# DefTruth/CUDA-Learn-Notes

Measured on NVIDIA H100. Metric: hgemm_tflops, higher is better.
Workload: dtype f16 (fp32 accumulate)

## Files before the change

### cuda-learn-notes_b200/csrc/hgemm_wgmma.cu

```cuda
#include "abi_common.cuh"
#include "ptx.cuh"

namespace b200k {

namespace gemm {
constexpr int BM = 128, BN = 256, STAGES = 4, THREADS = 384, GROUP_M = 16;
constexpr int STG_BYTES = 16384;
}

template <int DT_, bool A_MN_, bool B_MN_>
struct GemmCfg {
  static constexpr int DT = DT_;
  static constexpr bool A_MN = A_MN_, B_MN = B_MN_;
  static constexpr int ES = DT == 2 ? 4 : 2;
  static constexpr int BK = 128 / ES;
  static constexpr int KSTEP = DT == 2 ? 8 : 16;
  static constexpr int A_BYTES = gemm::BM * BK * ES;
  static constexpr int B_BYTES = gemm::BN * BK * ES;
  static constexpr int STAGE_BYTES = A_BYTES + B_BYTES;
  static constexpr int SMEM_BYTES = gemm::STAGES * STAGE_BYTES + 2 * gemm::STG_BYTES + 1024 + 2 * gemm::STAGES * 8;
  static_assert(!(DT == 2 && (A_MN || B_MN)), "tf32 wgmma reads K-major operands only");
  static_assert(SMEM_BYTES <= 232448, "more shared memory than an H100 block may use");
};

template <class Cfg>
__device__ __forceinline__ void gemm_mma_kblock(float* d, uint32_t sA, uint32_t sB, int cw) {
  constexpr int STEPS = Cfg::BK / Cfg::KSTEP;
#pragma unroll
  for (int k = 0; k < STEPS; ++k) {
    const uint64_t da = Cfg::A_MN ? wgmma_desc(sA + cw * 64 * Cfg::BK * Cfg::ES + k * 2048, 64 * Cfg::BK * Cfg::ES, 1024)
                                  : wgmma_desc(sA + cw * 64 * 128 + k * 32, 16, 1024);
    const uint64_t db = Cfg::B_MN ? wgmma_desc(sB + k * 2048, 64 * Cfg::BK * Cfg::ES, 1024) : wgmma_desc(sB + k * 32, 16, 1024);
    wgmma_ss<Cfg::DT, 256, Cfg::A_MN, Cfg::B_MN>(d, da, db, 1);
  }
}

template <class Cfg>
__device__ __forceinline__ void gemm_store_tile(const float* d, const CUtensorMap* tmC, uint32_t stg, int cw, int row0,
                                                int col0) {
  constexpr int SLICES = Cfg::DT == 2 ? 4 : 2, JS = 32 / SLICES, JB = JS / 2;
  const int t = threadIdx.x & 127, lane = t & 31, warp = t / 32;
  const bool leader = t == 0;
#pragma unroll
  for (int sl = 0; sl < SLICES; ++sl) {
    if (leader) tma_store_wait_read<0>();
    named_bar_sync(1 + cw, 128);
    if constexpr (Cfg::DT == 2) {
      const int q = lane & 3;
#pragma unroll
      for (int jj = 0; jj < JS; ++jj) {
        const int j = sl * JS + jj;
#pragma unroll
        for (int h = 0; h < 2; ++h) {
          const int r = warp * 16 + 8 * h + lane / 4;
          const int chunk = 2 * (jj % JB) + q / 2;
          const uint32_t a = stg + (jj / JB) * 8192 + r * 128 + ((chunk ^ (r & 7)) << 4) + (q & 1) * 8;
          asm volatile("st.shared.v2.f32 [%0], {%1, %2};" ::"r"(a), "f"(d[4 * j + 2 * h]), "f"(d[4 * j + 2 * h + 1])
                       : "memory");
        }
      }
    } else {
      const int m = lane / 8, r = warp * 16 + 8 * (m & 1) + (lane & 7);
#pragma unroll
      for (int jj = 0; jj < JS; jj += 2) {
        const int j = sl * JS + jj, chunk = jj % JB + (m >> 1);
        const uint32_t a = stg + (jj / JB) * 8192 + r * 128 + ((chunk ^ (r & 7)) << 4);
        uint32_t p[4];
#pragma unroll
        for (int i = 0; i < 4; ++i)
          p[i] = Cfg::DT == 1 ? pack_bf162(d[4 * j + 2 * i], d[4 * j + 2 * i + 1])
                              : pack_half2(d[4 * j + 2 * i], d[4 * j + 2 * i + 1]);
        stmatrix_x4(a, p[0], p[1], p[2], p[3]);
      }
    }
    fence_proxy_async_smem();
    named_bar_sync(1 + cw, 128);
    if (leader) {
      const int c = col0 + sl * (gemm::BN / SLICES);
      tma_store_2d(tmC, stg, c, row0);
      tma_store_2d(tmC, stg + 8192, c + 128 / Cfg::ES, row0);
      tma_store_commit();
    }
  }
}

template <class Cfg>
__global__ void __launch_bounds__(gemm::THREADS, 1)
    hgemm_wgmma_kernel(const __grid_constant__ CUtensorMap tmA, const __grid_constant__ CUtensorMap tmB,
                       const __grid_constant__ CUtensorMap tmC, int K, int tiles_m, int tiles_n) {
  using namespace gemm;
  extern __shared__ uint8_t smem_raw[];
  const uint32_t base = (smem_u32(smem_raw) + 1023) & ~1023u;
  const uint32_t stg0 = base + STAGES * Cfg::STAGE_BYTES;
  const uint32_t full0 = stg0 + 2 * STG_BYTES, empty0 = full0 + STAGES * 8;
  const int wg = threadIdx.x / 128;

  const int tile = blockIdx.x, width = GROUP_M * tiles_n, g = tile / width, first_m = g * GROUP_M;
  const int gsz = min(tiles_m - first_m, GROUP_M);
  const int tm = first_m + (tile % width) % gsz, tn = (tile % width) / gsz;
  const int nkb = (K + Cfg::BK - 1) / Cfg::BK;

  if (threadIdx.x == 0) {
    for (int s = 0; s < STAGES; ++s) {
      mbar_init(full0 + 8 * s, 1);
      mbar_init(empty0 + 8 * s, 2);
    }
    fence_mbar_init();
  }
  __syncthreads();

  if (wg == 0) {
    if (threadIdx.x == 0) {
      tma_prefetch_desc(&tmA);
      tma_prefetch_desc(&tmB);
      for (int kb = 0; kb < nkb; ++kb) {
        const int s = kb % STAGES;
        if (kb >= STAGES) mbar_wait_nocall(empty0 + 8 * s, ((kb / STAGES) - 1) & 1);
        const uint32_t bar = full0 + 8 * s, sA = base + s * Cfg::STAGE_BYTES, sB = sA + Cfg::A_BYTES;
        mbar_arrive_expect_tx(bar, Cfg::STAGE_BYTES);
        if constexpr (Cfg::A_MN) {
#pragma unroll
          for (int c = 0; c < BM / 64; ++c)
            tma_load_2d(sA + c * 64 * Cfg::BK * Cfg::ES, &tmA, bar, tm * BM + c * 64, kb * Cfg::BK, kPolicyEvictNormal);
        } else {
          tma_load_2d(sA, &tmA, bar, kb * Cfg::BK, tm * BM, kPolicyEvictNormal);
        }
        if constexpr (Cfg::B_MN) {
#pragma unroll
          for (int c = 0; c < BN / 64; ++c)
            tma_load_2d(sB + c * 64 * Cfg::BK * Cfg::ES, &tmB, bar, tn * BN + c * 64, kb * Cfg::BK, kPolicyEvictNormal);
        } else {
          tma_load_2d(sB, &tmB, bar, kb * Cfg::BK, tn * BN, kPolicyEvictNormal);
        }
      }
    }
    return;
  }

  const int cw = wg - 1, t = threadIdx.x & 127;
  const bool leader = t == 0;
  if (leader) tma_prefetch_desc(&tmC);
  float d[128];
#pragma unroll
  for (int i = 0; i < 128; ++i) d[i] = 0.f;
  for (int kb = 0; kb < nkb; ++kb) {
    const int s = kb % STAGES;
    mbar_wait_nocall(full0 + 8 * s, (kb / STAGES) & 1);
    const uint32_t sA = base + s * Cfg::STAGE_BYTES, sB = sA + Cfg::A_BYTES;
    fence_regs<128>(d);
    wgmma_fence();
    gemm_mma_kblock<Cfg>(d, sA, sB, cw);
    wgmma_commit();
    wgmma_wait<1>();
    fence_regs<128>(d);
    if (kb > 0 && leader) mbar_arrive(empty0 + 8 * ((kb - 1) % STAGES));
  }
  wgmma_wait<0>();
  fence_regs<128>(d);
  gemm_store_tile<Cfg>(d, &tmC, stg0 + cw * STG_BYTES, cw, tm * BM + cw * 64, tn * BN);
  if (leader) tma_store_wait_all<0>();
}

template <class Cfg>
static int launch_gemm(const void* A, const void* B, void* C, int64_t M, int64_t N, int64_t K, cudaStream_t s,
                       const DeviceInfo& di) {
  using namespace gemm;
  auto tmap = [](CUtensorMap* m, const void* p, int64_t rows, int64_t cols, uint32_t box_rows, uint32_t box_cols) {
    const uint64_t dims[2] = {uint64_t(cols), uint64_t(rows)}, strides[1] = {uint64_t(cols) * Cfg::ES};
    const uint32_t box[2] = {box_cols, box_rows};
    return make_tmap(m, p, Cfg::ES, 2, dims, strides, box);
  };
  CUtensorMap tmA, tmB, tmC;
  int rc = Cfg::A_MN ? tmap(&tmA, A, K, M, Cfg::BK, 64) : tmap(&tmA, A, M, K, BM, Cfg::BK);
  if (rc) return rc;
  rc = Cfg::B_MN ? tmap(&tmB, B, K, N, Cfg::BK, 64) : tmap(&tmB, B, N, K, BN, Cfg::BK);
  if (rc) return rc;
  if ((rc = tmap(&tmC, C, M, N, 64, 128 / Cfg::ES))) return rc;
  const int64_t tiles_m = (M + BM - 1) / BM, tiles_n = (N + BN - 1) / BN, tiles = tiles_m * tiles_n;
  if (tiles > INT32_MAX) return set_error(B200K_ESHAPE, "GEMM too large: %lld tiles", (long long)tiles);
  auto kern = hgemm_wgmma_kernel<Cfg>;
  if ((rc = ensure_dynamic_smem(reinterpret_cast<const void*>(kern), di.device, Cfg::SMEM_BYTES))) return rc;
  kern<<<unsigned(tiles), THREADS, Cfg::SMEM_BYTES, s>>>(tmA, tmB, tmC, int(K), int(tiles_m), int(tiles_n));
  B200K_CHECK_CUDA(cudaGetLastError());
  return B200K_OK;
}

template <int DT>
static int gemm_dispatch(const char* who, const void* A, const void* B, void* C, int64_t M, int64_t N, int64_t K,
                         int b_is_nk, int variant, void* stream, int a_is_km = 0) {
  constexpr int PACK = (DT == 2) ? 4 : 8;
  if (!A || !B || !C) return set_error(B200K_EARG, "%s: null pointer", who);
  if (reinterpret_cast<uintptr_t>(C) & 15) return set_error(B200K_EALIGN, "%s: C (%p) must be 16-byte aligned", who, C);
  if (M < 1 || N < 1 || K < 1 || M > INT32_MAX || N > INT32_MAX || K > INT32_MAX)
    return set_error(B200K_ESHAPE, "%s: M,N,K must be in [1, 2^31) (got %lld,%lld,%lld)", who, (long long)M, (long long)N,
                     (long long)K);
  if ((K % PACK) || (N % PACK))
    return set_error(B200K_ESHAPE, "%s: K and N must be multiples of %d (16-byte rows), got K=%lld N=%lld", who, PACK,
                     (long long)K, (long long)N);
  if (a_is_km && DT == 2) return set_error(B200K_EDTYPE, "%s: A stored as [K,M] is built for f16 / bf16 only", who);
  if (a_is_km && (M % PACK))
    return set_error(B200K_ESHAPE, "%s: M must be a multiple of %d when A is stored as [K,M]", who, PACK);
  const int v = variant & 0xff;
  if (v < B200K_HGEMM_AUTO || v > B200K_HGEMM_2CTA_512x256)
    return set_error(B200K_EARG, "%s: variant %d unknown", who, v);
  DeviceInfo di;
  int rc = get_device_info(&di);
  if (rc) return rc;
  cudaStream_t s = static_cast<cudaStream_t>(stream);
  const bool nn = (b_is_nk == 0);
  if constexpr (DT == 2) {
    if (!nn) return launch_gemm<GemmCfg<2, false, false>>(A, B, C, M, N, K, s, di);
    void* bt = nullptr;
    B200K_CHECK_CUDA(cudaMallocAsync(&bt, size_t(K) * size_t(N) * 4, s));
    rc = b200k_mat_transpose_f32(B, bt, K, N, stream);
    if (!rc) rc = launch_gemm<GemmCfg<2, false, false>>(A, bt, C, M, N, K, s, di);
    cudaError_t e = cudaFreeAsync(bt, s);
    if (!rc && e != cudaSuccess) rc = set_error(B200K_ECUDA, "cudaFreeAsync failed: %s", cudaGetErrorString(e));
    return rc;
  } else {
    if (a_is_km)
      return nn ? launch_gemm<GemmCfg<DT, true, true>>(A, B, C, M, N, K, s, di)
                : launch_gemm<GemmCfg<DT, true, false>>(A, B, C, M, N, K, s, di);
    return nn ? launch_gemm<GemmCfg<DT, false, true>>(A, B, C, M, N, K, s, di)
              : launch_gemm<GemmCfg<DT, false, false>>(A, B, C, M, N, K, s, di);
  }
}

}

extern "C" int b200k_hgemm_f16(const void* A, const void* B, void* C, int64_t M, int64_t N, int64_t K, int b_is_nk,
                               int variant, void* stream) {
  return b200k::gemm_dispatch<0>("b200k_hgemm_f16", A, B, C, M, N, K, b_is_nk, variant, stream);
}

extern "C" int b200k_gemm_ex(const void* A, const void* B, void* C, int64_t M, int64_t N, int64_t K, int a_is_km, int b_is_nk,
                             int dtype, int variant, void* stream) {
  switch (dtype) {
    case B200K_F16: return b200k::gemm_dispatch<0>("b200k_gemm_ex(f16)", A, B, C, M, N, K, b_is_nk, variant, stream, a_is_km);
    case B200K_BF16: return b200k::gemm_dispatch<1>("b200k_gemm_ex(bf16)", A, B, C, M, N, K, b_is_nk, variant, stream, a_is_km);
    case B200K_F32: return b200k::gemm_dispatch<2>("b200k_gemm_ex(tf32)", A, B, C, M, N, K, b_is_nk, variant, stream, a_is_km);
    default: return b200k::set_error(B200K_EDTYPE, "b200k_gemm_ex: dtype %d not supported (f16, bf16, f32-as-tf32)", dtype);
  }
}

extern "C" int b200k_gemm(const void* A, const void* B, void* C, int64_t M, int64_t N, int64_t K, int b_is_nk, int dtype,
                          int variant, void* stream) {
  switch (dtype) {
    case B200K_F16: return b200k::gemm_dispatch<0>("b200k_gemm(f16)", A, B, C, M, N, K, b_is_nk, variant, stream);
    case B200K_BF16: return b200k::gemm_dispatch<1>("b200k_gemm(bf16)", A, B, C, M, N, K, b_is_nk, variant, stream);
    case B200K_F32: return b200k::gemm_dispatch<2>("b200k_gemm(tf32)", A, B, C, M, N, K, b_is_nk, variant, stream);
    default: return b200k::set_error(B200K_EDTYPE, "b200k_gemm: dtype %d not supported (f16, bf16, f32-as-tf32)", dtype);
  }
}
```

### cuda-learn-notes_b200/csrc/ptx.cuh

```cuda
#pragma once
#include <cstdint>
#include <cuda.h>
#include <cuda_bf16.h>
#include <cuda_fp16.h>
#include <cuda_runtime.h>

namespace b200k {

#ifndef B200K_SPIN_LIMIT_CYCLES
#define B200K_SPIN_LIMIT_CYCLES (10LL * 1000 * 1000 * 1000)
#endif

__device__ __forceinline__ uint32_t smem_u32(const void* p) {
  return static_cast<uint32_t>(__cvta_generic_to_shared(p));
}
__device__ __forceinline__ void named_bar_sync(uint32_t id, uint32_t nthreads) {
  asm volatile("bar.sync %0, %1;" ::"r"(id), "r"(nthreads) : "memory");
}

__device__ __forceinline__ void mbar_init(uint32_t bar, uint32_t count) {
  asm volatile("mbarrier.init.shared::cta.b64 [%0], %1;" ::"r"(bar), "r"(count) : "memory");
}
__device__ __forceinline__ void fence_mbar_init() {
  asm volatile("fence.mbarrier_init.release.cluster;" ::: "memory");
}
__device__ __forceinline__ void fence_proxy_async_smem() {
  asm volatile("fence.proxy.async.shared::cta;" ::: "memory");
}
__device__ __forceinline__ void mbar_arrive(uint32_t bar) {
  asm volatile("mbarrier.arrive.shared::cta.b64 _, [%0];" ::"r"(bar) : "memory");
}
__device__ __forceinline__ void mbar_arrive_expect_tx(uint32_t bar, uint32_t bytes) {
  asm volatile("mbarrier.arrive.expect_tx.shared::cta.b64 _, [%0], %1;" ::"r"(bar), "r"(bytes) : "memory");
}
__device__ __forceinline__ uint32_t mbar_try_wait(uint32_t bar, uint32_t parity) {
  uint32_t ok;
  asm volatile(
      "{\n\t"
      ".reg .pred P1;\n\t"
      "mbarrier.try_wait.parity.shared::cta.b64 P1, [%1], %2;\n\t"
      "selp.u32 %0, 1, 0, P1;\n\t"
      "}"
      : "=r"(ok)
      : "r"(bar), "r"(parity)
      : "memory");
  return ok;
}
static __device__ __noinline__ void mbar_timeout_trap(uint32_t bar, uint32_t parity) {
  printf("[b200k] mbarrier wait timed out: block (%d,%d) thread %d bar 0x%x parity %u\n", blockIdx.x, blockIdx.y,
         threadIdx.x, bar, parity);
  __trap();
}
__device__ __forceinline__ void mbar_wait(uint32_t bar, uint32_t parity) {
  if (mbar_try_wait(bar, parity)) return;
  long long t0 = clock64();
  while (!mbar_try_wait(bar, parity)) {
    if (clock64() - t0 > B200K_SPIN_LIMIT_CYCLES) mbar_timeout_trap(bar, parity);
  }
}
__device__ __forceinline__ void mbar_wait_nocall(uint32_t bar, uint32_t parity) {
  if (mbar_try_wait(bar, parity)) return;
  long long t0 = clock64();
  while (!mbar_try_wait(bar, parity)) {
    if (clock64() - t0 > B200K_SPIN_LIMIT_CYCLES) asm volatile("trap;");
  }
}

__device__ __forceinline__ void tma_prefetch_desc(const CUtensorMap* m) {
  asm volatile("prefetch.tensormap [%0];" ::"l"(reinterpret_cast<uint64_t>(m)) : "memory");
}
constexpr uint64_t kPolicyEvictNormal = 0x1000000000000000ull;
constexpr uint64_t kPolicyEvictFirst = 0x12F0000000000000ull;

__device__ __forceinline__ void tma_load_2d(uint32_t dst_smem, const CUtensorMap* m, uint32_t bar, int32_t c0,
                                            int32_t c1, uint64_t policy) {
  asm volatile(
      "cp.async.bulk.tensor.2d.shared::cluster.global.mbarrier::complete_tx::bytes.L2::cache_hint"
      " [%0], [%1, {%3, %4}], [%2], %5;" ::"r"(dst_smem),
      "l"(reinterpret_cast<uint64_t>(m)), "r"(bar), "r"(c0), "r"(c1), "l"(policy)
      : "memory");
}
__device__ __forceinline__ void tma_load_3d(uint32_t dst_smem, const CUtensorMap* m, uint32_t bar, int32_t c0,
                                            int32_t c1, int32_t c2, uint64_t policy) {
  asm volatile(
      "cp.async.bulk.tensor.3d.shared::cluster.global.mbarrier::complete_tx::bytes.L2::cache_hint"
      " [%0], [%1, {%3, %4, %5}], [%2], %6;" ::"r"(dst_smem),
      "l"(reinterpret_cast<uint64_t>(m)), "r"(bar), "r"(c0), "r"(c1), "r"(c2), "l"(policy)
      : "memory");
}
__device__ __forceinline__ void tma_store_2d(const CUtensorMap* m, uint32_t src_smem, int32_t c0, int32_t c1) {
  asm volatile("cp.async.bulk.tensor.2d.global.shared::cta.bulk_group [%0, {%2, %3}], [%1];" ::"l"(
                   reinterpret_cast<uint64_t>(m)),
               "r"(src_smem), "r"(c0), "r"(c1)
               : "memory");
}
__device__ __forceinline__ void tma_store_commit() { asm volatile("cp.async.bulk.commit_group;" ::: "memory"); }
template <int N>
__device__ __forceinline__ void tma_store_wait_read() {
  asm volatile("cp.async.bulk.wait_group.read %0;" ::"n"(N) : "memory");
}
template <int N>
__device__ __forceinline__ void tma_store_wait_all() {
  asm volatile("cp.async.bulk.wait_group %0;" ::"n"(N) : "memory");
}
__device__ __forceinline__ void stmatrix_x4(uint32_t addr, uint32_t r0, uint32_t r1, uint32_t r2, uint32_t r3) {
  asm volatile("stmatrix.sync.aligned.m8n8.x4.shared.b16 [%0], {%1, %2, %3, %4};" ::"r"(addr), "r"(r0), "r"(r1), "r"(r2),
               "r"(r3)
               : "memory");
}

__device__ __forceinline__ uint64_t wgmma_desc(uint32_t smem_addr, uint32_t lbo, uint32_t sbo) {
  return uint64_t((smem_addr & 0x3FFFF) >> 4) | (uint64_t(lbo >> 4) << 16) | (uint64_t(sbo >> 4) << 32) | (1ull << 62);
}
__device__ __forceinline__ void wgmma_fence() { asm volatile("wgmma.fence.sync.aligned;" ::: "memory"); }
__device__ __forceinline__ void wgmma_commit() { asm volatile("wgmma.commit_group.sync.aligned;" ::: "memory"); }
template <int N>
__device__ __forceinline__ void wgmma_wait() { asm volatile("wgmma.wait_group.sync.aligned %0;" ::"n"(N) : "memory"); }
template <int N>
__device__ __forceinline__ void fence_regs(float* d) {
#pragma unroll
  for (int i = 0; i < N; ++i) asm volatile("" : "+f"(d[i])::"memory");
}

#define B200K_ACC8(i) \
  "+f"(d[i]), "+f"(d[i + 1]), "+f"(d[i + 2]), "+f"(d[i + 3]), "+f"(d[i + 4]), "+f"(d[i + 5]), "+f"(d[i + 6]), "+f"(d[i + 7])
#define B200K_ACC32(i) B200K_ACC8(i), B200K_ACC8(i + 8), B200K_ACC8(i + 16), B200K_ACC8(i + 24)
#define B200K_ACC64 B200K_ACC32(0)
#define B200K_ACC128 B200K_ACC64, B200K_ACC32(32)
#define B200K_ACC192 B200K_ACC128, B200K_ACC32(64)
#define B200K_ACC256 B200K_ACC192, B200K_ACC32(96)
#define B200K_PH64 \
  "%0, %1, %2, %3, %4, %5, %6, %7, %8, %9, %10, %11, %12, %13, %14, %15, " \
  "%16, %17, %18, %19, %20, %21, %22, %23, %24, %25, %26, %27, %28, %29, %30, %31"
#define B200K_PH128 \
  B200K_PH64 ", %32, %33, %34, %35, %36, %37, %38, %39, %40, %41, %42, %43, %44, %45, %46, %47, " \
  "%48, %49, %50, %51, %52, %53, %54, %55, %56, %57, %58, %59, %60, %61, %62, %63"
#define B200K_PH192 \
  B200K_PH128 ", %64, %65, %66, %67, %68, %69, %70, %71, %72, %73, %74, %75, %76, %77, %78, %79, " \
  "%80, %81, %82, %83, %84, %85, %86, %87, %88, %89, %90, %91, %92, %93, %94, %95"
#define B200K_PH256 \
  B200K_PH192 ", %96, %97, %98, %99, %100, %101, %102, %103, %104, %105, %106, %107, %108, %109, %110, %111, " \
  "%112, %113, %114, %115, %116, %117, %118, %119, %120, %121, %122, %123, %124, %125, %126, %127"
#define B200K_WGMMA(shape, type, acc, scale, ops) \
  "{\n.reg .pred p;\nsetp.ne.b32 p, " scale ", 0;\n" \
  "wgmma.mma_async.sync.aligned." shape ".f32." type " {" acc "}, " ops ";\n}\n"
#define B200K_SS(type, n, scale, ops) \
  asm volatile(B200K_WGMMA("m64n" #n "k16", type, B200K_PH##n, scale, ops) \
               : B200K_ACC##n \
               : "l"(da), "l"(db), "r"(scale_d), "n"(TA), "n"(TB))
#define B200K_RS(type, n, scale, ops) \
  asm volatile(B200K_WGMMA("m64n" #n "k16", type, B200K_PH##n, scale, ops) \
               : B200K_ACC##n \
               : "r"(a[0]), "r"(a[1]), "r"(a[2]), "r"(a[3]), "l"(db), "r"(scale_d), "n"(TB))
#define B200K_F16_OR_BF16(op, ...) \
  if constexpr (DT == 0) \
    op("f16.f16", __VA_ARGS__); \
  else \
    op("bf16.bf16", __VA_ARGS__)

template <int DT, int N, int TA, int TB>
__device__ __forceinline__ void wgmma_ss(float* d, uint64_t da, uint64_t db, int scale_d) {
  static_assert(N == 64 || N == 128 || N == 256, "wgmma_ss: N must be 64, 128 or 256");
  static_assert(DT == 0 || DT == 1 || (DT == 2 && N == 256 && TA == 0 && TB == 0),
                "wgmma_ss: f16 / bf16, or tf32 with N = 256 and K-major operands");
  if constexpr (DT == 2) {
    asm volatile(B200K_WGMMA("m64n256k8", "tf32.tf32", B200K_PH256, "%130", "%128, %129, p, 1, 1")
                 : B200K_ACC256
                 : "l"(da), "l"(db), "r"(scale_d));
  } else if constexpr (N == 64) {
    B200K_F16_OR_BF16(B200K_SS, 64, "%34", "%32, %33, p, 1, 1, %35, %36");
  } else if constexpr (N == 128) {
    B200K_F16_OR_BF16(B200K_SS, 128, "%66", "%64, %65, p, 1, 1, %67, %68");
  } else {
    B200K_F16_OR_BF16(B200K_SS, 256, "%130", "%128, %129, p, 1, 1, %131, %132");
  }
}
template <int DT, int N, int TB>
__device__ __forceinline__ void wgmma_rs(float* d, const uint32_t* a, uint64_t db, int scale_d) {
  static_assert(N == 64 || N == 128 || N == 192 || N == 256, "wgmma_rs: N must be 64, 128, 192 or 256");
  static_assert(DT == 0 || DT == 1, "wgmma_rs: f16 or bf16");
  if constexpr (N == 64) {
    B200K_F16_OR_BF16(B200K_RS, 64, "%37", "{%32, %33, %34, %35}, %36, p, 1, 1, %38");
  } else if constexpr (N == 128) {
    B200K_F16_OR_BF16(B200K_RS, 128, "%69", "{%64, %65, %66, %67}, %68, p, 1, 1, %70");
  } else if constexpr (N == 192) {
    B200K_F16_OR_BF16(B200K_RS, 192, "%101", "{%96, %97, %98, %99}, %100, p, 1, 1, %102");
  } else {
    B200K_F16_OR_BF16(B200K_RS, 256, "%133", "{%128, %129, %130, %131}, %132, p, 1, 1, %134");
  }
}
#undef B200K_ACC8
#undef B200K_ACC32
#undef B200K_ACC64
#undef B200K_ACC128
#undef B200K_ACC192
#undef B200K_ACC256
#undef B200K_PH64
#undef B200K_PH128
#undef B200K_PH192
#undef B200K_PH256
#undef B200K_WGMMA
#undef B200K_SS
#undef B200K_RS
#undef B200K_F16_OR_BF16

__device__ __forceinline__ uint32_t pack_half2(float lo, float hi) {
  __half2 h = __floats2half2_rn(lo, hi);
  return *reinterpret_cast<uint32_t*>(&h);
}
__device__ __forceinline__ uint32_t pack_bf162(float lo, float hi) {
  __nv_bfloat162 h = __floats2bfloat162_rn(lo, hi);
  return *reinterpret_cast<uint32_t*>(&h);
}

}
```

Before: 760.6.

## Pair CTAs in 2-CTA clusters and multicast shared B tiles via TMA

Launches the GEMM in 2-CTA clusters where both CTAs share the same N tile and adjacent M tiles. Each CTA loads half of the B tile and multicasts it to both CTAs, which halves per-CTA global/L2 traffic for B. Empty barriers now take arrivals from both CTAs' consumers through cross-CTA mbarrier arrives. Phantom CTAs pad an odd tiles_m and skip the A load and the store. The cost is cross-CTA synchronisation coupling, a producer drain loop before exit, and a changed tile rasterization.

```diff
diff --git a/cuda-learn-notes_b200/csrc/hgemm_wgmma.cu b/cuda-learn-notes_b200/csrc/hgemm_wgmma.cu
--- a/cuda-learn-notes_b200/csrc/hgemm_wgmma.cu
+++ b/cuda-learn-notes_b200/csrc/hgemm_wgmma.cu
@@ -85,7 +85,7 @@
 }
 
 template <class Cfg>
-__global__ void __launch_bounds__(gemm::THREADS, 1)
+__global__ void __cluster_dims__(2, 1, 1) __launch_bounds__(gemm::THREADS, 1)
     hgemm_wgmma_kernel(const __grid_constant__ CUtensorMap tmA, const __grid_constant__ CUtensorMap tmB,
                        const __grid_constant__ CUtensorMap tmC, int K, int tiles_m, int tiles_n) {
   using namespace gemm;
@@ -95,19 +95,21 @@
   const uint32_t full0 = stg0 + 2 * STG_BYTES, empty0 = full0 + STAGES * 8;
   const int wg = threadIdx.x / 128;
 
-  const int tile = blockIdx.x, width = GROUP_M * tiles_n, g = tile / width, first_m = g * GROUP_M;
-  const int gsz = min(tiles_m - first_m, GROUP_M);
-  const int tm = first_m + (tile % width) % gsz, tn = (tile % width) / gsz;
+  const uint32_t rank = cluster_ctarank();
+  const int pairs_m = (tiles_m + 1) / 2, p = blockIdx.x / 2, width = (GROUP_M / 2) * tiles_n, g = p / width;
+  const int first_pm = g * (GROUP_M / 2), gsz = min(pairs_m - first_pm, GROUP_M / 2);
+  const int tm = 2 * (first_pm + (p % width) % gsz) + int(rank), tn = (p % width) / gsz;
+  const bool phantom = tm == tiles_m;
   const int nkb = (K + Cfg::BK - 1) / Cfg::BK;
 
   if (threadIdx.x == 0) {
     for (int s = 0; s < STAGES; ++s) {
       mbar_init(full0 + 8 * s, 1);
-      mbar_init(empty0 + 8 * s, 2);
+      mbar_init(empty0 + 8 * s, 4);
     }
     fence_mbar_init();
   }
-  __syncthreads();
+  cluster_sync_after_init();
 
   if (wg == 0) {
     if (threadIdx.x == 0) {
@@ -117,28 +119,39 @@
         const int s = kb % STAGES;
         if (kb >= STAGES) mbar_wait_nocall(empty0 + 8 * s, ((kb / STAGES) - 1) & 1);
         const uint32_t bar = full0 + 8 * s, sA = base + s * Cfg::STAGE_BYTES, sB = sA + Cfg::A_BYTES;
-        mbar_arrive_expect_tx(bar, Cfg::STAGE_BYTES);
-        if constexpr (Cfg::A_MN) {
-#pragma unroll
-          for (int c = 0; c < BM / 64; ++c)
-            tma_load_2d(sA + c * 64 * Cfg::BK * Cfg::ES, &tmA, bar, tm * BM + c * 64, kb * Cfg::BK, kPolicyEvictNormal);
-        } else {
-          tma_load_2d(sA, &tmA, bar, kb * Cfg::BK, tm * BM, kPolicyEvictNormal);
+        mbar_arrive_expect_tx(bar, phantom ? Cfg::B_BYTES : Cfg::STAGE_BYTES);
+        if (!phantom) {
+          if constexpr (Cfg::A_MN) {
+#pragma unroll
+            for (int c = 0; c < BM / 64; ++c)
+              tma_load_2d(sA + c * 64 * Cfg::BK * Cfg::ES, &tmA, bar, tm * BM + c * 64, kb * Cfg::BK, kPolicyEvictNormal);
+          } else {
+            tma_load_2d(sA, &tmA, bar, kb * Cfg::BK, tm * BM, kPolicyEvictNormal);
+          }
         }
         if constexpr (Cfg::B_MN) {
 #pragma unroll
-          for (int c = 0; c < BN / 64; ++c)
-            tma_load_2d(sB + c * 64 * Cfg::BK * Cfg::ES, &tmB, bar, tn * BN + c * 64, kb * Cfg::BK, kPolicyEvictNormal);
+          for (int c = int(rank) * (BN / 128); c < int(rank + 1) * (BN / 128); ++c)
+            tma_load_2d_mc(sB + c * 64 * Cfg::BK * Cfg::ES, &tmB, bar, tn * BN + c * 64, kb * Cfg::BK, 0b11,
+                           kPolicyEvictNormal);
         } else {
-          tma_load_2d(sB, &tmB, bar, kb * Cfg::BK, tn * BN, kPolicyEvictNormal);
+          tma_load_2d_mc(sB + rank * (BN / 2) * 128, &tmB, bar, kb * Cfg::BK, tn * BN + int(rank) * (BN / 2), 0b11,
+                         kPolicyEvictNormal);
         }
       }
+      for (int kb = max(nkb, STAGES); kb < nkb + STAGES; ++kb)
+        mbar_wait_nocall(empty0 + 8 * (kb % STAGES), ((kb / STAGES) - 1) & 1);
     }
     return;
   }
 
   const int cw = wg - 1, t = threadIdx.x & 127;
   const bool leader = t == 0;
+  const uint32_t peer_empty0 = mapa_shared(empty0, rank ^ 1);
+  auto release = [&](int s) {
+    mbar_arrive(empty0 + 8 * s);
+    mbar_arrive_cluster(peer_empty0 + 8 * s);
+  };
   if (leader) tma_prefetch_desc(&tmC);
   float d[128];
 #pragma unroll
@@ -153,11 +166,12 @@
     wgmma_commit();
     wgmma_wait<1>();
     fence_regs<128>(d);
-    if (kb > 0 && leader) mbar_arrive(empty0 + 8 * ((kb - 1) % STAGES));
+    if (kb > 0 && leader) release((kb - 1) % STAGES);
   }
   wgmma_wait<0>();
   fence_regs<128>(d);
-  gemm_store_tile<Cfg>(d, &tmC, stg0 + cw * STG_BYTES, cw, tm * BM + cw * 64, tn * BN);
+  if (leader) release((nkb - 1) % STAGES);
+  if (!phantom) gemm_store_tile<Cfg>(d, &tmC, stg0 + cw * STG_BYTES, cw, tm * BM + cw * 64, tn * BN);
   if (leader) tma_store_wait_all<0>();
 }
 
@@ -173,10 +187,10 @@
   CUtensorMap tmA, tmB, tmC;
   int rc = Cfg::A_MN ? tmap(&tmA, A, K, M, Cfg::BK, 64) : tmap(&tmA, A, M, K, BM, Cfg::BK);
   if (rc) return rc;
-  rc = Cfg::B_MN ? tmap(&tmB, B, K, N, Cfg::BK, 64) : tmap(&tmB, B, N, K, BN, Cfg::BK);
+  rc = Cfg::B_MN ? tmap(&tmB, B, K, N, Cfg::BK, 64) : tmap(&tmB, B, N, K, BN / 2, Cfg::BK);
   if (rc) return rc;
   if ((rc = tmap(&tmC, C, M, N, 64, 128 / Cfg::ES))) return rc;
-  const int64_t tiles_m = (M + BM - 1) / BM, tiles_n = (N + BN - 1) / BN, tiles = tiles_m * tiles_n;
+  const int64_t tiles_m = (M + BM - 1) / BM, tiles_n = (N + BN - 1) / BN, tiles = 2 * ((tiles_m + 1) / 2) * tiles_n;
   if (tiles > INT32_MAX) return set_error(B200K_ESHAPE, "GEMM too large: %lld tiles", (long long)tiles);
   auto kern = hgemm_wgmma_kernel<Cfg>;
   if ((rc = ensure_dynamic_smem(reinterpret_cast<const void*>(kern), di.device, Cfg::SMEM_BYTES))) return rc;
diff --git a/cuda-learn-notes_b200/csrc/ptx.cuh b/cuda-learn-notes_b200/csrc/ptx.cuh
--- a/cuda-learn-notes_b200/csrc/ptx.cuh
+++ b/cuda-learn-notes_b200/csrc/ptx.cuh
@@ -18,6 +18,20 @@
   asm volatile("bar.sync %0, %1;" ::"r"(id), "r"(nthreads) : "memory");
 }
 
+__device__ __forceinline__ uint32_t cluster_ctarank() {
+  uint32_t r;
+  asm("mov.u32 %0, %%cluster_ctarank;" : "=r"(r));
+  return r;
+}
+__device__ __forceinline__ uint32_t mapa_shared(uint32_t addr, uint32_t rank) {
+  uint32_t r;
+  asm("mapa.shared::cluster.u32 %0, %1, %2;" : "=r"(r) : "r"(addr), "r"(rank));
+  return r;
+}
+__device__ __forceinline__ void cluster_sync_after_init() {
+  asm volatile("barrier.cluster.arrive.relaxed.aligned;\n\tbarrier.cluster.wait.aligned;" ::: "memory");
+}
+
 __device__ __forceinline__ void mbar_init(uint32_t bar, uint32_t count) {
   asm volatile("mbarrier.init.shared::cta.b64 [%0], %1;" ::"r"(bar), "r"(count) : "memory");
 }
@@ -29,6 +43,9 @@
 }
 __device__ __forceinline__ void mbar_arrive(uint32_t bar) {
   asm volatile("mbarrier.arrive.shared::cta.b64 _, [%0];" ::"r"(bar) : "memory");
+}
+__device__ __forceinline__ void mbar_arrive_cluster(uint32_t cluster_bar) {
+  asm volatile("mbarrier.arrive.shared::cluster.b64 _, [%0];" ::"r"(cluster_bar) : "memory");
 }
 __device__ __forceinline__ void mbar_arrive_expect_tx(uint32_t bar, uint32_t bytes) {
   asm volatile("mbarrier.arrive.expect_tx.shared::cta.b64 _, [%0], %1;" ::"r"(bar), "r"(bytes) : "memory");
@@ -78,6 +95,14 @@
       "cp.async.bulk.tensor.2d.shared::cluster.global.mbarrier::complete_tx::bytes.L2::cache_hint"
       " [%0], [%1, {%3, %4}], [%2], %5;" ::"r"(dst_smem),
       "l"(reinterpret_cast<uint64_t>(m)), "r"(bar), "r"(c0), "r"(c1), "l"(policy)
+      : "memory");
+}
+__device__ __forceinline__ void tma_load_2d_mc(uint32_t dst_smem, const CUtensorMap* m, uint32_t bar, int32_t c0,
+                                               int32_t c1, uint16_t cta_mask, uint64_t policy) {
+  asm volatile(
+      "cp.async.bulk.tensor.2d.shared::cluster.global.mbarrier::complete_tx::bytes.multicast::cluster.L2::cache_hint"
+      " [%0], [%1, {%3, %4}], [%2], %5, %6;" ::"r"(dst_smem),
+      "l"(reinterpret_cast<uint64_t>(m)), "r"(bar), "r"(c0), "r"(c1), "h"(cta_mask), "l"(policy)
       : "memory");
 }
 __device__ __forceinline__ void tma_load_3d(uint32_t dst_smem, const CUtensorMap* m, uint32_t bar, int32_t c0,
```

Result: no change. 766.2 (median of 6 runs) (+0.7%).
